# toposware/schnorr-sig

Hardware: AMD Instinct MI355X
Metric: Schnorr verifications/sec, 2^20-sig batch, 1/2/4/8 MI355X; bit-exact vs CPU (higher is better)
Workload: dtype u64

## Files before the change

### include/schnorr_sig_amd.h

```cpp
#ifndef SCHNORR_SIG_AMD_H
#define SCHNORR_SIG_AMD_H

#include <stddef.h>
#include <stdint.h>

#ifdef __cplusplus
extern "C" {
#endif

#define SSA_SIGNATURE_LENGTH 81
#define SSA_AFFINE_PK_LENGTH 96
#define SSA_SCALAR_LENGTH 32
#define SSA_PUBLIC_KEY_LENGTH 49
#define SSA_DIGEST_LENGTH 32
#define SSA_PARAMS_LENGTH 2816

#define SSA_OK 0
#define SSA_INVALID_PUBLIC_KEY 1
#define SSA_INVALID_SIGNATURE 2
#define SSA_MALFORMED 3

#define SSA_ERR_ARG (-1)
#define SSA_ERR_HIP (-2)
#define SSA_ERR_PARAMS (-3)
// ... 230 lines not shown

int ssa_multi_verify_batch_msm(ssa_multi *m, const uint8_t *sigs, const uint8_t *pks, const uint8_t *pk_inf,
                               const uint8_t *msgs, const uint64_t *msg_off, size_t msg_stride, size_t msg_len,
                               size_t n, const uint8_t *coeffs);

#define SSA_MSM_PARTIAL_WORDS 24
#define SSA_MSM_RECORD_MAGIC 0x5353415245430004ull
int ssa_verify_batch_msm_partial_device(ssa_ctx *ctx, const uint8_t *d_sigs, const uint8_t *d_pks,
                                        const uint8_t *d_pk_inf, const uint8_t *d_msgs, const uint64_t *d_msg_off,
                                        size_t msg_stride, size_t msg_len, size_t n, const uint8_t *d_coeffs,
                                        uint32_t coeff_bytes, uint64_t *d_partial_out);
int ssa_verify_batch_msm_partial(ssa_ctx *ctx, const uint8_t *sigs, const uint8_t *pks, const uint8_t *pk_inf,
                                 const uint8_t *msgs, const uint64_t *msg_off, size_t msg_stride, size_t msg_len,
                                 size_t n, const uint8_t *coeffs, uint64_t out24[SSA_MSM_PARTIAL_WORDS]);
int ssa_msm_combine_device(ssa_ctx *ctx, const uint64_t *d_parts24, size_t k, uint32_t *d_verdict_out);
int ssa_msm_combine(ssa_ctx *ctx, const uint64_t *parts24, size_t k);

#define SSA_ABI_VERSION 5
int ssa_abi_version(void);

int ssa_debug_arith(ssa_ctx *ctx, int op, const uint64_t *a, const uint64_t *b, size_t n,
                    size_t a_stride, size_t b_stride, uint64_t *out, size_t out_stride);
int ssa_debug_fault_after_chunk(ssa_ctx *ctx, int chunk);
int ssa_debug_table_read(ssa_ctx *ctx, int which, uint64_t first_row, uint64_t n, uint64_t *rows_out);
int ssa_debug_table_xor(ssa_ctx *ctx, int which, uint64_t row, uint32_t word, uint64_t mask);
int ssa_debug_corrupt_table_builds(int n);
int ssa_debug_keytab_xor(ssa_keyset *ks, ssa_keycache *kc, int what, uint64_t key, uint32_t word, uint64_t mask);
int ssa_debug_keytab_read(ssa_keyset *ks, ssa_keycache *kc, int what, uint64_t key, uint64_t *words_out);
int ssa_debug_tail_plan(unsigned waves, unsigned pieces, unsigned gens, int uniform, unsigned min_main, size_t n,
                        uint32_t flags, uint32_t out[14]);
int ssa_debug_screen_plan(size_t n, uint32_t coeff_bytes, uint64_t out[8]);
int ssa_debug_screen_segments(ssa_ctx *ctx, uint32_t k);
int ssa_debug_dedup_device(ssa_ctx *ctx, const uint8_t *d_pks, const uint8_t *d_pk_inf, size_t n,
                           uint32_t *d_key_idx_out, uint64_t out[2]);
int ssa_debug_dedup_config(ssa_ctx *ctx, double max_distinct_ratio, uint32_t probe_bound);
int ssa_debug_keycache_plan(uint64_t capacity, uint64_t held, uint64_t u, uint64_t m, uint32_t *plan_out);
int ssa_debug_chacha20(ssa_ctx *ctx, const uint8_t key[32], const uint8_t nonce[12], uint32_t counter0,
                       size_t n_blocks, uint8_t *out);
int ssa_bench_fpmul(ssa_ctx *ctx, int variant, double *fpmul_per_s);

#ifdef __cplusplus
}
#endif
#endif
```

### schnorr-sig_amd/__init__.py

```python
import ctypes as C
import os

import numpy as np

_HERE = os.path.dirname(os.path.abspath(__file__))
LIB_PATH = os.environ.get("SSA_LIB") or os.path.join(_HERE, "csrc", "libschnorr_sig_amd.so")

SCALAR_LENGTH = 32
PRIVATE_KEY_LENGTH = 32
BASEFIELD_LENGTH = 48
PUBLIC_KEY_LENGTH = 49
AFFINE_PUBLIC_KEY_LENGTH = 96
KEY_PAIR_LENGTH = 32
SIGNATURE_LENGTH = 81
KEYED_SIGNATURE_LENGTH = 130

OK, INVALID_PUBLIC_KEY, INVALID_SIGNATURE, MALFORMED = 0, 1, 2, 3
ERR_ARG, ERR_HIP, ERR_PARAMS, ERR_NO_DEVICE, ERR_TABLE = -1, -2, -3, -4, -5
TABLE_COMB, TABLE_CT = 0, 1
SELFCHECK_FIELDS = ("rows", "bad", "first_bad", "ctab_rows", "ctab_bad", "ctab_first_bad", "builds", "bits")
FLAG_CHECK_TORSION = 1
FLAG_FORCE_LANE = 2
FLAG_FORCE_COOP = 4
FLAG_SIG_FLAG_BYTE = 8
# ... 169 lines not shown
        "ssa_sign_many_indexed": (i32, [vp, vp, vp, vp, vp, vp, sz, sz, sz, u32, vp]),
        "ssa_sign_many_indexed_device": (i32, [vp, vp, vp, vp, vp, vp, sz, sz, sz, u32, vp, vp]),
        "ssa_ctx_selfcheck": (i32, [vp, u32, u64p]),
        "ssa_debug_table_read": (i32, [vp, i32, C.c_uint64, C.c_uint64, vp]),
        "ssa_debug_table_xor": (i32, [vp, i32, C.c_uint64, u32, C.c_uint64]),
        "ssa_debug_corrupt_table_builds": (i32, [i32]),
        "ssa_keyset_selfcheck": (i32, [vp, u32, vp, u64p]),
        "ssa_keycache_selfcheck": (i32, [vp, u32, u64p]),
        "ssa_debug_keytab_xor": (i32, [vp, vp, i32, C.c_uint64, u32, C.c_uint64]),
        "ssa_debug_keytab_read": (i32, [vp, vp, i32, C.c_uint64, vp]),
        "ssa_keygen_sign_many_rng": (i32, [vp, vp, vp, vp, sz, sz, sz, u32, vp, vp]),
        "ssa_keygen_sign_many_rng_device": (i32, [vp, vp, vp, vp, sz, sz, sz, u32, vp, vp]),
        "ssa_sign_many_indexed_rng": (i32, [vp, vp, vp, vp, vp, sz, sz, sz, u32, vp]),
        "ssa_sign_many_indexed_rng_device": (i32, [vp, vp, vp, vp, vp, sz, sz, sz, u32, vp, vp]),
        "ssa_signer_set_generate": (i32, [vp, sz, C.POINTER(vp)]),
        "ssa_signer_set_secret_keys": (i32, [vp, vp]),
        "ssa_debug_pin_rng": (i32, [vp, vp]),
        "ssa_debug_draw_scalars": (i32, [vp, vp, sz, vp]),
    }
    for name, (res, args) in sigs.items():
        fn = getattr(lib, name)
        fn.restype = res
        fn.argtypes = args
    got = lib.ssa_abi_version()
    if got != ABI_VERSION:
        raise ImportError("schnorr_sig_amd: %s has ABI version %d, this binding was written for %d -- rebuild "
                          "(python -c 'import __graft_entry__ as g; g.build(force=True)')" % (LIB_PATH, got, ABI_VERSION))
    return lib, list(sigs)


ABI_VERSION = 5
MSM_PARTIAL_WORDS = 24
MSM_RECORD_MAGIC = 0x5353415245430004
_lib, ABI_SYMBOLS = _load()


def _check(rc, what):
    if rc < 0:
        raise RuntimeError("%s failed: %s (%d)" % (what, _lib.ssa_strerror(rc).decode(), rc))
    return rc


def _np_u8(a, cols=None):
    a = np.ascontiguousarray(a, dtype=np.uint8)
    if cols is not None:
        a = a.reshape(-1, cols)
    return a


def _ptr(a):
    return None if a is None else C.c_void_p(a.ctypes.data)
# ... 573 lines not shown
        cnt = C.c_uint64(0)
        _check(_lib.ssa_ctx_read_timing(self._ctx, kernel.encode(), C.byref(avg), C.byref(cnt)),
               "ssa_ctx_read_timing")
        return avg.value, int(cnt.value)

    def host_path_probe(self, sigs_t, pks_t, msgs_t, n, reps=3):
        import time
        hs, hp, hm = (t[:n].cpu().numpy() for t in (sigs_t, pks_t, msgs_t))
        st, nf = self.verify_many(hs, hp, hm, check_torsion=False, mode="lane", sig_flag_byte=True)
        t0 = time.perf_counter()
        for _ in range(reps):
            st, nf = self.verify_many(hs, hp, hm, check_torsion=False, mode="lane", sig_flag_byte=True)
        dt = (time.perf_counter() - t0) / reps
        verdict = self.verify_batch_msm(hs, hp, hm)
        t0 = time.perf_counter()
        for _ in range(reps):
            verdict = self.verify_batch_msm(hs, hp, hm)
        dt_msm = (time.perf_counter() - t0) / reps
        return {"entry_point": "ssa_verify_many (host buffers in pageable memory, copied through the library's page-locked "
                               "bounce buffers, uploads in chunks overlapped with the hash kernel)",
                "ms_per_batch": dt * 1e3, "verifications_per_sec": n / dt, "rejected": int(nf),
                "verify_batch_msm_ms_per_batch": dt_msm * 1e3, "verify_batch_msm_signatures_per_sec": n / dt_msm,
                "verify_batch_msm_verdict": int(verdict)}

    def debug_arith(self, op, a, b, out_cols):
        a = np.ascontiguousarray(a, dtype=np.uint64)
        b = np.ascontiguousarray(b, dtype=np.uint64) if b is not None else None
        n = a.shape[0]
        out = np.zeros((n, out_cols), dtype=np.uint64)
        _check(_lib.ssa_debug_arith(self._ctx, op, _ptr(a), _ptr(b), n, a.shape[1],
                                    b.shape[1] if b is not None else 0, _ptr(out), out_cols), "ssa_debug_arith")
        return out

    def bench_fpmul(self, variant):
        v = C.c_double(0)
        _check(_lib.ssa_bench_fpmul(self._ctx, variant, C.byref(v)), "ssa_bench_fpmul")
        return v.value


def debug_corrupt_table_builds(n):
    _check(_lib.ssa_debug_corrupt_table_builds(int(n)), "ssa_debug_corrupt_table_builds")


KEYCHECK_DEEP, KEYCHECK_REPAIR = 1, 2
KEYCHECK_FIELDS = ("keys_checked", "keys_bad", "first_bad_key", "ladder_entries_checked", "comb_rows_checked",
                   "keys_rebuilt_and_compared", "combs_skipped", "rows_repaired")
# ... 193 lines not shown
        m = _np_u8(msgs)
        off = np.ascontiguousarray(offsets, dtype=np.uint64) if offsets is not None else None
        stride = mlen = 0 if off is not None else m.shape[1]
        inf = _np_u8(pk_inf) if pk_inf is not None else None
        c = _np_u8(coeffs, 32) if coeffs is not None else None
        return _check(_lib.ssa_multi_verify_batch_msm(self._m, _ptr(sigs), _ptr(pks), _ptr(inf), _ptr(m), _ptr(off),
                                                      stride, mlen, n, _ptr(c)), "ssa_multi_verify_batch_msm")


_default_engine = None


def debug_tail_plan(waves, n, check_torsion=False, pieces=5, gens=1, uniform=False, min_main=0):
    out = np.zeros(14, dtype=np.uint32)
    flags = 1 if check_torsion else 0
    _check(_lib.ssa_debug_tail_plan(int(waves), int(pieces), int(gens), int(bool(uniform)), int(min_main), int(n), flags,
                                    out.ctypes.data), "ssa_debug_tail_plan")

    def dec(d):
        d = int(d)
        return (d & 1, bool(d & 2), bool(d & 4), (d >> 8) & 0xff, (d >> 16) & 0xff)
    return {"n_pieces": int(out[0]), "tail_groups": int(out[1]), "main_blocks": int(out[2]), "grid_blocks": int(out[3]),
            "pieces": [dec(out[4 + k]) for k in range(int(out[0]))], "whole": [dec(out[12]), dec(out[13])]}


def debug_screen_plan(n, coeff_bytes=0):
    out = np.zeros(8, dtype=np.uint64)
    _check(_lib.ssa_debug_screen_plan(int(n), int(coeff_bytes), out.ctypes.data), "ssa_debug_screen_plan")
    keys = ("segments", "segment_lanes", "window_bits", "windows", "r_windows", "buckets_per_window", "slices",
            "total_segments")
    return {k: int(v) for k, v in zip(keys, out)}


def default_engine():
    global _default_engine
    if _default_engine is None:
        _default_engine = Engine(0)
    return _default_engine


class PublicKey:

    def __init__(self, affine96, is_identity=False):
        b = bytes(affine96)
        if len(b) != AFFINE_PUBLIC_KEY_LENGTH:
            raise ValueError("PublicKey needs 96 bytes of affine coordinates")
# ... 437 lines not shown
```

### schnorr-sig_amd/csrc/ssa_api.hip

```cpp
#define SSA_KERNELS_DEFINE 1
#include "ssa_ctx.hpp"
#include "ssa_keycache.hpp"

#include <sys/random.h>

#include <atomic>
#include <climits>
#include <functional>
#include <initializer_list>
#include <memory>
#include <mutex>
#include <thread>

static const unsigned char k_default_params[SSA_PARAMS_LENGTH] = {
#include "../params/params_default.inc"
};

extern "C" const char *ssa_strerror(int rc) {
    switch (rc) {
        case SSA_OK: return "ok";
        case SSA_INVALID_PUBLIC_KEY: return "The public key is not an element of the prime subgroup.";
        case SSA_INVALID_SIGNATURE: return "The signature is invalid or was incorrectly computed.";
        case SSA_MALFORMED: return "malformed input (the reference would panic)";
        case SSA_ERR_ARG: return "invalid argument";
// ... 136 lines not shown
    int v = 0;
    if (env_int(name, INT_MIN, INT_MAX, v) && std::find(set.begin(), set.end(), v) != set.end()) knob = (T)v;
}
static void env_flag(const char *name, bool &knob) {
    int v = 0;
    if (env_int(name, INT_MIN, INT_MAX, v)) knob = v != 0;
}

static void ctx_read_env(ssa_ctx *ctx, uint32_t *gtab_bits, uint64_t *hbm_budget_bytes) {
    CtxKnobs &k = ctx->knobs;
    if (env_u64("SSA_COOP_MAX_N", 0, UINT64_MAX, k.coop_max_n)) k.coop_max_n_torsion = k.coop_max_n;
    env_u64("SSA_MSM_SMALL_MAX", 0, UINT64_MAX, k.msm_small_max);
    env_one_of("SSA_VERIFY_BLOCK", {64, 128, 256}, k.verify_block);
    env_u64("SSA_LANE_SLICE", 256, UINT64_MAX, k.lane_slice);
    env_u64("SSA_MSM_SLICE", 256, (uint64_t)1 << 23, k.msm_slice);
    env_int("SSA_MSM_TREE_GROUP", 2, 64, k.msm_tree_group);
    env_int("SSA_TAIL_PIECES", 0, VP_MAX, k.tail_pieces);
    env_int("SSA_TAIL_GENS", 1, 8, k.tail_gens);
    env_flag("SSA_TAIL_UNIFORM", k.tail_uniform);
    env_int("SSA_TAIL_MIN_MAIN", INT_MIN, INT_MAX, k.tail_min_main);
    env_flag("SSA_TAIL_REVERSED", k.tail_reversed);
    env_int("SSA_TAIL_WAVES", INT_MIN, INT_MAX, k.tail_waves_override);
    env_flag("SSA_MSM_OVERLAP", k.msm_overlap);
    env_int("SSA_PIPELINE_CHUNKS", 1, 8, k.pipeline_chunks);
    env_flag("SSA_TWO_STREAMS", ctx->two_streams);
    uint64_t mb = 0;
    if (*hbm_budget_bytes == 0 && env_u64("SSA_HBM_BUDGET_MB", 0, UINT64_MAX, mb)) *hbm_budget_bytes = mb << 20;
    if (*gtab_bits == 0) env_one_of("SSA_GTAB_BITS", {16, 20, 22, 24}, *gtab_bits);
}

static int ctx_create(ssa_ctx **out, int device, const void *params, size_t params_len, uint32_t gtab_bits,
                      uint64_t hbm_budget_bytes, const CtxKnobs *inherit) {
    if (!out) return SSA_ERR_ARG;
    *out = nullptr;
    if (gtab_bits != 0 && gtab_bits != 16 && gtab_bits != 20 && gtab_bits != 22 && gtab_bits != 24) return SSA_ERR_ARG;
    int count = 0;
    if (hipGetDeviceCount(&count) != hipSuccess || count == 0) return SSA_ERR_NO_DEVICE;
    if (device < 0 || device >= count) return SSA_ERR_ARG;
    DevParams hp;
    if (params) {
        if (params_len != sizeof(DevParams)) return SSA_ERR_PARAMS;
        std::memcpy(&hp, params, sizeof hp);
    } else {
        std::memcpy(&hp, k_default_params, sizeof hp);
    }
    const bool is_default = std::memcmp(&hp, k_default_params, sizeof hp) == 0;
    if (int rc = validate_params(hp)) return rc;
    hp.flags = 0;
    bool small_mds = true;
    for (int i = 0; i < 144; i++) small_mds = small_mds && hp.mds[i] <= 0xffffffffull;
    if (small_mds) hp.flags |= PRM_FLAG_SMALL_MDS;
    bool tiny_mds = true;
    for (int i = 0; i < 144; i++) tiny_mds = tiny_mds && hp.mds[i] < 0x10000ull;
    if (tiny_mds) hp.flags |= PRM_FLAG_TINY_MDS;
    HIP_TRY(hipSetDevice(device));
    std::unique_ptr<ssa_ctx, decltype(&ssa_ctx_destroy)> guard(new ssa_ctx(), ssa_ctx_destroy);
    ssa_ctx *ctx = guard.get();
    ctx->device = device;
    ctx->default_params = is_default;
    if (inherit) ctx->knobs = *inherit;
    else ctx_read_env(ctx, &gtab_bits, &hbm_budget_bytes);
    HIP_TRY(hipStreamCreateWithFlags(&ctx->own_stream, hipStreamNonBlocking));
    HIP_TRY(hipStreamCreateWithFlags(&ctx->copy_stream, hipStreamNonBlocking));
    for (auto &st : ctx->hash_stream) HIP_TRY(hipStreamCreateWithFlags(&st, hipStreamNonBlocking));
    HIP_TRY(hipEventCreateWithFlags(&ctx->pipe_start, hipEventDisableTiming));
    HIP_TRY(hipEventCreateWithFlags(&ctx->order_ev, hipEventDisableTiming));
    for (int i = 0; i < 8; i++) {
        HIP_TRY(hipEventCreateWithFlags(&ctx->copy_done[i], hipEventDisableTiming));
        HIP_TRY(hipEventCreateWithFlags(&ctx->hash_done[i], hipEventDisableTiming));
    }
    ctx->stream = ctx->own_stream;
    if (!inherit) {
        hipDeviceProp_t prop;
        int occ = 0;
        if (hipGetDeviceProperties(&prop, device) == hipSuccess &&
            hipOccupancyMaxActiveBlocksPerMultiprocessor(&occ, ssa_k_verify, 256, 0) == hipSuccess && occ > 0)
            ctx->knobs.verify_waves = (unsigned)prop.multiProcessorCount * (unsigned)occ * 4u;
        (void)hipGetLastError();
        if (ctx->knobs.tail_waves_override) ctx->knobs.verify_waves = ctx->knobs.tail_waves_override;
    }
    HIP_TRY(hipMalloc((void **)&ctx->d_params, sizeof(DevParams)));
    HIP_TRY(hipMemcpy(ctx->d_params, &hp, sizeof hp, hipMemcpyHostToDevice));
    ctx->h_params = hp;
    if (hbm_budget_bytes == 0) {
        size_t free_b = 0, total_b = 0;
        if (hipMemGetInfo(&free_b, &total_b) != hipSuccess) free_b = 0;
        hbm_budget_bytes = free_b / 10;
    }
    ctx->hbm_budget = hbm_budget_bytes;
    static const u32 k_widths[4] = {24, 22, 20, 16};
    bool bad_table = false;
    for (u32 wbits : k_widths) {
        if (gtab_bits ? wbits > gtab_bits : (wbits > 16 && gtab_bytes(wbits) > hbm_budget_bytes)) continue;
// ... 14 lines not shown
    *out = guard.release();
    return 0;
}

extern "C" int ssa_ctx_create_ex(ssa_ctx **out, int device, const void *params, size_t params_len, uint32_t gtab_bits,
                                 uint64_t hbm_budget_bytes) {
    return ctx_create(out, device, params, params_len, gtab_bits, hbm_budget_bytes, nullptr);
}

extern "C" int ssa_ctx_create(ssa_ctx **out, int device, const void *params, size_t params_len) {
    return ssa_ctx_create_ex(out, device, params, params_len, 0u, 0ull);
}

ssa_ctx *ssa_internal_twin(ssa_ctx *ctx) {
    if (ctx->is_twin || !ctx->two_streams) return nullptr;
    if (!ctx->twin) {
        DevParams hp = ctx->h_params;
        hp.flags = 0;
        if (ctx_create(&ctx->twin, ctx->device, &hp, sizeof hp, ctx->gtab_bits, ctx->hbm_budget, &ctx->knobs) != 0) {
            ctx->two_streams = false;
            return nullptr;
        }
        ctx->twin->is_twin = true;
    }
    ctx->twin->knobs = ctx->knobs;
    return ctx->twin;
}

template <class T, class F>
static void orphan_handles(std::vector<T *> &v, F &&release) {
    for (T *h : v) {
        release(h);
        h->ctx = nullptr;
    }
    v.clear();
}

extern "C" void ssa_ctx_destroy(ssa_ctx *ctx) {
    if (!ctx) return;
    (void)hipSetDevice(ctx->device);
    if (ctx->stream) (void)hipStreamSynchronize(ctx->stream);
    if (ctx->twin) {
        ssa_ctx_destroy(ctx->twin);
        ctx->twin = nullptr;
    }
    orphan_handles(ctx->keysets, [](ssa_keyset *ks) { ks->release_all(); });
    orphan_handles(ctx->signer_sets, [](ssa_signer_set *ss) { ss->wipe_release(); });
    orphan_handles(ctx->keycaches, [](ssa_keycache *kc) { kc->release_all(); });
    for (auto &kv : ctx->timed)
        for (auto &t : kv.second) {
            (void)hipEventDestroy(t.start);
            (void)hipEventDestroy(t.stop);
        }
    for_each_devbuf(ctx, [](DevBuf &b) { b.release(); });
    for_each_hostbuf(ctx, [](HostBuf &b) { b.release(); });
    if (ctx->d_params) (void)hipFree(ctx->d_params);
    gtab_release(ctx->gtab_share);
    ctx->gtab_share = nullptr;
    ctx->d_gtab = nullptr;
    for (auto &ev : ctx->copy_done)
        if (ev) (void)hipEventDestroy(ev);
    for (auto &ev : ctx->hash_done)
        if (ev) (void)hipEventDestroy(ev);
    if (ctx->pipe_start) (void)hipEventDestroy(ctx->pipe_start);
    if (ctx->order_ev) (void)hipEventDestroy(ctx->order_ev);
    for (auto &st : ctx->hash_stream)
        if (st) (void)hipStreamDestroy(st);
    if (ctx->copy_stream) (void)hipStreamDestroy(ctx->copy_stream);
// ... 1063 lines not shown
            std::vector<uint64_t> off;
            const HostBatch s = b.slice(lo, cnt, off);
            rcs[r] = ssa_verify_batch_msm_partial(m->ctxs[r], s.sigs, s.pks, s.pk_inf, s.msgs, s.msg_off, msg_stride, msg_len,
                                                  cnt, coeffs ? coeffs + 32 * lo : nullptr, &parts[24 * r]);
        });
    }
    for (auto &t : threads) t.join();
    for (size_t r = 0; r < world; r++)
        if (rcs[r] != 0) return rcs[r];
    return ssa_msm_combine(m->ctxs[0], parts.data(), world);
}

extern "C" int ssa_debug_corrupt_table_builds(int n) {
    if (n < 0) return SSA_ERR_ARG;
    g_corrupt_builds.store(n);
    return 0;
}

extern "C" int ssa_debug_fault_after_chunk(ssa_ctx *ctx, int chunk) {
    if (!ctx) return SSA_ERR_ARG;
    ctx->fault_after_chunk = chunk;
    return 0;
}

extern "C" int ssa_debug_arith(ssa_ctx *ctx, int op, const uint64_t *a, const uint64_t *b, size_t n,
                               size_t a_stride, size_t b_stride, uint64_t *out, size_t out_stride) {
    if (!ctx || !a || !out || n == 0 || op < 0 || op > 18) return SSA_ERR_ARG;
    if ((op == 0 || op == 3 || op == 4 || op == 5 || (op >= 7 && op != 18)) && !b) return SSA_ERR_ARG;
    if (op == 18 && (a_stride < 2 || out_stride < 6)) return SSA_ERR_ARG;
    if (op >= 15 && op <= 17) {
        if (a_stride < 20 || b_stride < 12 || out_stride < 19) return SSA_ERR_ARG;
        if (op != 16)
            for (size_t i = 0; i < n; i++)
                if (a[i * a_stride + 19] == 0 || a[i * a_stride + 19] > 64 || a[i * a_stride + 19] != a[19])
                    return SSA_ERR_ARG;
    }
    HostCall hc(ctx);
    const u64 *da = hc.in<u64>(ctx->st_aux, a, n * a_stride * 8), *db = b ? hc.in<u64>(ctx->st_aux2, b, n * b_stride * 8) : nullptr;
    u64 *d_out = (u64 *)hc.out(ctx->st_status, out, n * out_stride * 8);
    return hc.finish([&] {
        HIP_TRY(hipMemsetAsync(d_out, 0, n * out_stride * 8, ctx->stream));
        if (op == 7) {
            hipLaunchKernelGGL(ssa_k_debug_coop, dim3((unsigned)n), dim3(64), 0, ctx->stream, da, db, n, a_stride, b_stride,
                               d_out, out_stride);
        } else if (op == 4 || (op >= 15 && op <= 17)) {
            if (ctx->ws_tab.reserve(n * (size_t)(PTAB_ENTRIES * PTAB_ENTRY_U64) * sizeof(u64))) return SSA_ERR_HIP;
// ... 100 lines not shown
```

### schnorr-sig_amd/csrc/ssa_ctx.hpp

```cpp
#pragma once
#include "../../include/schnorr_sig_amd.h"
#include "ssa_kernels.hpp"

#include <hip/hip_runtime.h>

#include <algorithm>
#include <cstdio>
#include <cstdlib>
#include <cstring>
#include <map>
#include <mutex>
#include <string>
#include <thread>
#include <utility>
#include <vector>

using namespace ssa;

static inline bool ssa_debug_enabled() {
    static const bool on = std::getenv("SSA_DEBUG") != nullptr;
    return on;
}
#define HIP_TRY(expr)                                                                    \
    do {                                                                                 \
// ... 49 lines not shown
            (void)hipGetLastError();
            p = nullptr;
            return SSA_ERR_HIP;
        }
        cap = want;
        return 0;
    }
    void release() {
        if (p) (void)hipHostFree(p);
        p = nullptr;
        cap = 0;
    }
};

struct TimedLaunch {
    hipEvent_t start, stop;
};

constexpr double DEDUP_RATIO_NO_CHECK = 0.0, DEDUP_RATIO_CHECK = 1.0;
constexpr unsigned DEDUP_PROBE_BOUND = 128;

struct CtxKnobs {
    size_t pipeline_min_n = 1 << 17;
    unsigned pipeline_chunks = 8;
    size_t coop_max_n = 7680, coop_max_n_torsion = 10496;
    size_t msm_small_max = 3072;
    size_t lane_slice = (size_t)1 << 20, msm_slice = (size_t)1 << 23;
    bool msm_overlap = true;
    unsigned msm_tree_group = 16;
    unsigned verify_block = 256;
    unsigned verify_waves = 0;
    unsigned tail_pieces = 5;
    unsigned tail_gens = 1;
    bool tail_uniform = false;
    bool tail_reversed = false;
    unsigned tail_min_main = 0;
    unsigned tail_waves_override = 0;
    bool timing = false;
    unsigned screen_segs = 0;
    double dedup_ratio[2] = {DEDUP_RATIO_NO_CHECK, DEDUP_RATIO_CHECK};
    unsigned dedup_probe_bound = DEDUP_PROBE_BOUND;
};

#define SSA_CTX_DEVBUFS(X) \
    X(ws_h) X(ws_tab) X(ws_fail) \
     \
    X(st_sigs) X(st_pks) X(st_inf) X(st_msgs) X(st_off) X(st_status) X(st_aux) X(st_aux2) X(st_coeffs) \
// ... 8 lines not shown
     \
    X(scr_mask) X(scr_mark) X(scr_list) X(scr_blk) X(scr_cnt) \
     \
    X(dd_slots) X(dd_rep) X(dd_num) X(dd_reps) X(dd_idx) X(dd_blk) X(dd_stats) X(dd_pks) X(dd_inf) X(dd_kstatus) \
     \
    X(kc_found) X(kc_missrep) X(kc_blk) X(kc_lane_row) \
     \
    X(ctab) X(sg_sigs) X(sg_pks) \
    X(tc_out)            \
    X(kck_ws)            \
    X(dv_recs)           \
     \
    X(rng_seed) X(rng_scratch) \
     \
    X(tail_done) X(tail_park)

#define SSA_CTX_HOSTBUFS(X) X(pin_in) X(pin_coeffs) X(pin_out) X(pin_seed)

struct ssa_ctx {
    int device = 0;
    hipStream_t own_stream = nullptr;
    hipStream_t stream = nullptr;
    hipStream_t copy_stream = nullptr;
    hipEvent_t copy_done[8] = {};
    hipStream_t hash_stream[2] = {};
    hipEvent_t hash_done[8] = {};
    hipEvent_t pipe_start = nullptr;
    hipEvent_t order_ev = nullptr;
    CtxKnobs knobs;
    DevParams *d_params = nullptr;
    u64 *d_gtab = nullptr;
    struct SharedGtab *gtab_share = nullptr;
    uint32_t gtab_bits = 0;
    uint64_t hbm_budget = 0;
    DevParams h_params;
    ssa_ctx *twin = nullptr;
    bool is_twin = false, two_streams = true;
#define X(name) DevBuf name;
    SSA_CTX_DEVBUFS(X)
#undef X
#define X(name) HostBuf name;
    SSA_CTX_HOSTBUFS(X)
#undef X
    bool default_params = false;
    int fault_after_chunk = -1;
    uint64_t dedup_key[2] = {0, 0};
    bool dedup_key_set = false;
    bool ctab_ready = false;
    bool rng_pinned = false;
    uint8_t rng_pin[44] = {};
    std::map<std::string, std::vector<TimedLaunch>> timed;
    std::vector<struct ssa_keyset *> keysets;
    std::vector<struct ssa_signer_set *> signer_sets;
    std::vector<struct ssa_keycache *> keycaches;
};

template <class Ctx, class F>
static inline void for_each_devbuf(Ctx *c, F &&f) {
#define X(name) f(c->name);
    SSA_CTX_DEVBUFS(X)
// ... 272 lines not shown
        settled = rc == 0;
        return rc;
    }
};


int ssa_internal_hash_chunk(ssa_ctx *ctx, hipStream_t hs, const DevBatch &b, size_t cnt, uint64_t *d_h);

struct SideStreamDrain {
    ssa_ctx *armed = nullptr;
    void done() { armed = nullptr; }
    ~SideStreamDrain() {
        if (!armed) return;
        (void)hipStreamSynchronize(armed->copy_stream);
        for (auto &hs : armed->hash_stream) (void)hipStreamSynchronize(hs);
        (void)hipStreamSynchronize(armed->stream);
    }
};

struct PipelinedInputs : SideStreamDrain {
    StagedInputs s;
};

static inline size_t host_copy_threads() {
    static const size_t t = [] {
        const char *e = std::getenv("SSA_COPY_THREADS");
        const long v = e ? std::atol(e) : 8;
        return (size_t)(v < 1 ? 1 : v > 32 ? 32 : v);
    }();
    return t;
}
static inline void host_copy(void *dst, const void *src, size_t bytes) {
    constexpr size_t PIECE = 4u << 20;
    if (bytes <= 2 * PIECE || host_copy_threads() == 1) {
        std::memcpy(dst, src, bytes);
        return;
    }
    const size_t parts = bytes / PIECE < host_copy_threads() ? bytes / PIECE : host_copy_threads();
    const size_t per = (bytes / parts + 63) & ~(size_t)63;
    std::vector<std::thread> th;
    for (size_t t = 1; t < parts; t++) {
        const size_t lo = t * per, hi = t + 1 == parts ? bytes : (t + 1) * per;
        th.emplace_back([=] { std::memcpy((char *)dst + lo, (const char *)src + lo, hi - lo); });
    }
    std::memcpy(dst, src, per < bytes ? per : bytes);
    for (auto &x : th) x.join();
}

static inline int pipeline_fault_chunk(ssa_ctx *ctx) {
    const int k = ctx->fault_after_chunk;
    ctx->fault_after_chunk = -1;
    return k;
}

static inline int pipelined_upload_hash(ssa_ctx *ctx, const HostBatch &b, size_t n, PipelinedInputs &pin, bool *used) {
    const uint8_t *sigs = b.sigs, *pks = b.pks, *pk_inf = b.pk_inf, *msgs = b.msgs;
    const uint64_t *msg_off = b.msg_off;
    const size_t msg_stride = b.msg_stride, msg_len = b.msg_len;
    *used = false;
    const size_t mb = msgs_bytes(msg_off, msg_stride, msg_len, n);
    if (mb && !msgs) return SSA_ERR_ARG;
    auto al = [](size_t b) { return (b + 255) & ~(size_t)255; };
    const size_t o_pks = al(n * 81), o_msgs = o_pks + al(n * 96), o_inf = o_msgs + al(mb),
                 o_off = o_inf + al(pk_inf ? n : 0), total = o_off + al(msg_off ? (n + 1) * sizeof(uint64_t) : 0);
    if (ctx->pin_in.reserve(total)) return 0;
    u8 *h_sigs = (u8 *)ctx->pin_in.p, *h_pks = h_sigs + o_pks, *h_msgs = h_sigs + o_msgs, *h_inf = h_sigs + o_inf,
       *h_off = h_sigs + o_off;
    *used = true;
    if (ctx->st_sigs.reserve(n * 81) || ctx->st_pks.reserve(n * 96) || ctx->st_msgs.reserve(mb + 16) ||
        ctx->ws_h.reserve(n * 4 * sizeof(u64)) || (msg_off && ctx->st_off.reserve((n + 1) * sizeof(uint64_t))) ||
        (pk_inf && ctx->st_inf.reserve(n)))
        return SSA_ERR_HIP;
    HIP_TRY(hipEventRecord(ctx->pipe_start, ctx->stream));
    HIP_TRY(hipStreamWaitEvent(ctx->copy_stream, ctx->pipe_start, 0));
    for (auto &hs : ctx->hash_stream) HIP_TRY(hipStreamWaitEvent(hs, ctx->pipe_start, 0));
    pin.armed = ctx;
    const int fault_chunk = pipeline_fault_chunk(ctx);
    u8 *d_sigs = (u8 *)ctx->st_sigs.p, *d_pks = (u8 *)ctx->st_pks.p, *d_msgs = (u8 *)ctx->st_msgs.p;
    DevBatch &d = pin.s.batch;
    d = {d_sigs, d_pks, nullptr, {d_msgs, nullptr, msg_stride, msg_len}};
    if (msg_off) {
        host_copy(h_off, msg_off, (n + 1) * sizeof(uint64_t));
        HIP_TRY(hipMemcpyAsync(ctx->st_off.p, h_off, (n + 1) * sizeof(uint64_t), hipMemcpyHostToDevice, ctx->copy_stream));
        d.msgs.off = (const u64 *)ctx->st_off.p;
    }
    if (pk_inf) {
        host_copy(h_inf, pk_inf, n);
        HIP_TRY(hipMemcpyAsync(ctx->st_inf.p, h_inf, n, hipMemcpyHostToDevice, ctx->copy_stream));
        d.pk_inf = (const u8 *)ctx->st_inf.p;
    }
    const unsigned chunks = ctx->knobs.pipeline_chunks;
    for (unsigned c = 0; c < chunks; c++) {
        const size_t lo = n * c / chunks, hi = n * (c + 1) / chunks, cnt = hi - lo;
        if (cnt == 0) continue;
        host_copy(h_sigs + 81 * lo, sigs + 81 * lo, cnt * 81);
        HIP_TRY(hipMemcpyAsync(d_sigs + 81 * lo, h_sigs + 81 * lo, cnt * 81, hipMemcpyHostToDevice, ctx->copy_stream));
        host_copy(h_pks + 96 * lo, pks + 96 * lo, cnt * 96);
        HIP_TRY(hipMemcpyAsync(d_pks + 96 * lo, h_pks + 96 * lo, cnt * 96, hipMemcpyHostToDevice, ctx->copy_stream));
        const size_t m_lo = msg_off ? (size_t)msg_off[lo] : lo * msg_stride;
        const size_t m_hi = msg_off ? (size_t)msg_off[hi] : (hi == n ? mb : hi * msg_stride);
        if (m_hi > m_lo) {
            host_copy(h_msgs + m_lo, msgs + m_lo, m_hi - m_lo);
            HIP_TRY(hipMemcpyAsync(d_msgs + m_lo, h_msgs + m_lo, m_hi - m_lo, hipMemcpyHostToDevice, ctx->copy_stream));
        }
        HIP_TRY(hipEventRecord(ctx->copy_done[c], ctx->copy_stream));
        hipStream_t hs = ctx->hash_stream[c & 1u];
        HIP_TRY(hipStreamWaitEvent(hs, ctx->copy_done[c], 0));
        if (int rc = ssa_internal_hash_chunk(ctx, hs, d.slice(lo), cnt, (uint64_t *)ctx->ws_h.p + 4 * lo)) return rc;
        HIP_TRY(hipEventRecord(ctx->hash_done[c], hs));
        HIP_TRY(hipStreamWaitEvent(ctx->stream, ctx->hash_done[c], 0));
        if ((int)c == fault_chunk) return SSA_ERR_HIP;
    }
    return 0;
}

static inline StagedInputs slice_inputs(HostCall &hc, PipelinedInputs &pin, const HostBatch &b, size_t n,
                                        const uint8_t *coeffs, bool pipeline, bool pin_out) {
    ssa_ctx *ctx = hc.ctx;
    if (hc.ok() && pipeline && n >= ctx->knobs.pipeline_min_n && ctx->knobs.pipeline_chunks > 1 && !(pin_out && ctx->pin_out.reserve(n)) &&
        (!coeffs || ctx->pin_coeffs.reserve(n * 32) == 0)) {
        bool used = false;
        if (coeffs && ctx->st_coeffs.reserve(n * 32)) hc.rc = SSA_ERR_HIP;
        else hc.rc = pipelined_upload_hash(ctx, b, n, pin, &used);
        if (!hc.ok() || used) {
            StagedInputs s = pin.s;
            s.hashed = true;
            if (coeffs && hc.ok()) {
                host_copy(ctx->pin_coeffs.p, coeffs, n * 32);
                hc.step([&] {
                    HIP_TRY(hipMemcpyAsync(ctx->st_coeffs.p, ctx->pin_coeffs.p, n * 32, hipMemcpyHostToDevice, ctx->copy_stream));
                    HIP_TRY(hipEventRecord(ctx->pipe_start, ctx->copy_stream));
                    HIP_TRY(hipStreamWaitEvent(ctx->stream, ctx->pipe_start, 0));
                    return 0;
                });
                s.coeffs = (const u8 *)ctx->st_coeffs.p;
            }
            return s;
        }
    }
    StagedInputs s;
    s.batch.sigs = hc.in(ctx->st_sigs, b.sigs, n * 81);
    s.batch.pks = hc.in(ctx->st_pks, b.pks, n * 96);
    if (b.pk_inf) s.batch.pk_inf = hc.in(ctx->st_inf, b.pk_inf, n);
    s.batch.msgs = hc.msgs(b.msgs, b.msg_off, b.msg_stride, b.msg_len, n);
    if (coeffs) s.coeffs = hc.in(ctx->st_coeffs, coeffs, n * 32);
    return s;
}

template <class F>
static int status_host_one(ssa_ctx *ctx, const HostBatch &b, size_t n, const uint8_t *coeffs, bool pipeline, bool pin_out,
                           uint8_t *status_out, uint64_t *n_fail_out, F &&device_form) {
    HostCall hc(ctx);
    PipelinedInputs pin;
    const StagedInputs s = slice_inputs(hc, pin, b, n, coeffs, pipeline, pin_out);
    const bool through_pin = pin_out && s.hashed;
    u8 *d_status = hc.out(ctx->st_status, through_pin ? ctx->pin_out.p : status_out, n, 16);
    unsigned long long nf = 0, *d_fail = (unsigned long long *)ctx->ws_fail.p;
    hc.copy_back(&nf, d_fail, sizeof nf);
    if (int rc = hc.finish([&] { return device_form(s, d_status, d_fail); })) return rc;
// ... 89 lines not shown
```

Measured before the change: 30.61 million.

## Overlap host staging copies with uploads via persistent copy pool and ramped chunk plan

Replaces the per-call spawn-and-join threaded host memcpy with a persistent worker pool. All chunks' pageable-to-pinned copies are posted up front, so later chunks are staged while earlier chunks upload and hash. The uniform 8-chunk split becomes a plan with small, doubling leading chunks followed by 8 body chunks, which gets the first hash kernel started sooner. Coefficient and offset uploads are also chunked into the same pipeline. The cost is persistent threads, lock contention on a shared queue, and more HIP calls per batch.

```diff
diff --git a/include/schnorr_sig_amd.h b/include/schnorr_sig_amd.h
--- a/include/schnorr_sig_amd.h
+++ b/include/schnorr_sig_amd.h
@@ -276,6 +276,12 @@
 int ssa_debug_arith(ssa_ctx *ctx, int op, const uint64_t *a, const uint64_t *b, size_t n,
                     size_t a_stride, size_t b_stride, uint64_t *out, size_t out_stride);
 int ssa_debug_fault_after_chunk(ssa_ctx *ctx, int chunk);
+int ssa_debug_upload_plan(size_t n, uint32_t explicit_chunks, size_t first_lanes, uint64_t out[20]);
+int ssa_debug_copy_pool_create(void **pool_out);
+int ssa_debug_copy_pool_copy(void *pool, uint32_t threads, void *dst, const void *src, size_t bytes);
+int ssa_debug_copy_pool_workers(void *pool);
+void ssa_debug_copy_pool_destroy(void *pool);
+int ssa_debug_copy_workers(ssa_ctx *ctx);
 int ssa_debug_table_read(ssa_ctx *ctx, int which, uint64_t first_row, uint64_t n, uint64_t *rows_out);
 int ssa_debug_table_xor(ssa_ctx *ctx, int which, uint64_t row, uint32_t word, uint64_t mask);
 int ssa_debug_corrupt_table_builds(int n);
diff --git a/schnorr-sig_amd/__init__.py b/schnorr-sig_amd/__init__.py
--- a/schnorr-sig_amd/__init__.py
+++ b/schnorr-sig_amd/__init__.py
@@ -215,11 +215,26 @@
         fn = getattr(lib, name)
         fn.restype = res
         fn.argtypes = args
+    later = {
+        "ssa_debug_upload_plan": (i32, [sz, u32, sz, vp]),
+        "ssa_debug_copy_pool_create": (i32, [C.POINTER(vp)]),
+        "ssa_debug_copy_pool_copy": (i32, [vp, u32, vp, vp, sz]),
+        "ssa_debug_copy_pool_workers": (i32, [vp]),
+        "ssa_debug_copy_pool_destroy": (None, [vp]),
+        "ssa_debug_copy_workers": (i32, [vp]),
+    }
+    bound = list(sigs)
+    for name, (res, args) in later.items():
+        fn = getattr(lib, name, None)
+        if fn is not None:
+            fn.restype = res
+            fn.argtypes = args
+            bound.append(name)
     got = lib.ssa_abi_version()
     if got != ABI_VERSION:
         raise ImportError("schnorr_sig_amd: %s has ABI version %d, this binding was written for %d -- rebuild "
                           "(python -c 'import __graft_entry__ as g; g.build(force=True)')" % (LIB_PATH, got, ABI_VERSION))
-    return lib, list(sigs)
+    return lib, bound
 
 
 ABI_VERSION = 5
@@ -839,6 +854,9 @@
                 "ms_per_batch": dt * 1e3, "verifications_per_sec": n / dt, "rejected": int(nf),
                 "verify_batch_msm_ms_per_batch": dt_msm * 1e3, "verify_batch_msm_signatures_per_sec": n / dt_msm,
                 "verify_batch_msm_verdict": int(verdict)}
+
+    def debug_copy_workers(self):
+        return _check(_lib.ssa_debug_copy_workers(self._ctx), "ssa_debug_copy_workers")
 
     def debug_arith(self, op, a, b, out_cols):
         a = np.ascontiguousarray(a, dtype=np.uint64)
@@ -1078,6 +1096,37 @@
         return (d & 1, bool(d & 2), bool(d & 4), (d >> 8) & 0xff, (d >> 16) & 0xff)
     return {"n_pieces": int(out[0]), "tail_groups": int(out[1]), "main_blocks": int(out[2]), "grid_blocks": int(out[3]),
             "pieces": [dec(out[4 + k]) for k in range(int(out[0]))], "whole": [dec(out[12]), dec(out[13])]}
+
+
+def debug_upload_plan(n, chunks=0, first_lanes=0):
+    out = np.zeros(20, dtype=np.uint64)
+    _check(_lib.ssa_debug_upload_plan(int(n), int(chunks), int(first_lanes), out.ctypes.data), "ssa_debug_upload_plan")
+    k = int(out[0])
+    return {"bounds": [int(v) for v in out[3:4 + k]] if k else [], "ramp": int(out[1]), "pipeline_min_n": int(out[2])}
+
+
+class DebugCopyPool:
+
+    def __init__(self, threads=8):
+        self._pool = C.c_void_p()
+        self.threads = int(threads)
+        _check(_lib.ssa_debug_copy_pool_create(C.byref(self._pool)), "ssa_debug_copy_pool_create")
+
+    def copy(self, dst, src, nbytes=None):
+        nbytes = src.nbytes if nbytes is None else int(nbytes)
+        assert nbytes <= src.nbytes and nbytes <= dst.nbytes
+        _check(_lib.ssa_debug_copy_pool_copy(self._pool, self.threads, dst.ctypes.data, src.ctypes.data, nbytes),
+               "ssa_debug_copy_pool_copy")
+
+    def workers(self):
+        return _check(_lib.ssa_debug_copy_pool_workers(self._pool), "ssa_debug_copy_pool_workers")
+
+    def close(self):
+        if self._pool:
+            _lib.ssa_debug_copy_pool_destroy(self._pool)
+            self._pool = C.c_void_p()
+
+    __del__ = close
 
 
 def debug_screen_plan(n, coeff_bytes=0):
diff --git a/schnorr-sig_amd/csrc/ssa_api.hip b/schnorr-sig_amd/csrc/ssa_api.hip
--- a/schnorr-sig_amd/csrc/ssa_api.hip
+++ b/schnorr-sig_amd/csrc/ssa_api.hip
@@ -182,7 +182,9 @@
     env_flag("SSA_TAIL_REVERSED", k.tail_reversed);
     env_int("SSA_TAIL_WAVES", INT_MIN, INT_MAX, k.tail_waves_override);
     env_flag("SSA_MSM_OVERLAP", k.msm_overlap);
-    env_int("SSA_PIPELINE_CHUNKS", 1, 8, k.pipeline_chunks);
+    env_int("SSA_PIPELINE_CHUNKS", 1, (int)UPLOAD_MAX_CHUNKS, k.pipeline_chunks);
+    env_u64("SSA_PIPELINE_FIRST", 256, (uint64_t)1 << 20, k.pipeline_first);
+    env_int("SSA_COPY_THREADS", 1, 32, k.copy_threads);
     env_flag("SSA_TWO_STREAMS", ctx->two_streams);
     uint64_t mb = 0;
     if (*hbm_budget_bytes == 0 && env_u64("SSA_HBM_BUDGET_MB", 0, UINT64_MAX, mb)) *hbm_budget_bytes = mb << 20;
@@ -225,10 +227,8 @@
     for (auto &st : ctx->hash_stream) HIP_TRY(hipStreamCreateWithFlags(&st, hipStreamNonBlocking));
     HIP_TRY(hipEventCreateWithFlags(&ctx->pipe_start, hipEventDisableTiming));
     HIP_TRY(hipEventCreateWithFlags(&ctx->order_ev, hipEventDisableTiming));
-    for (int i = 0; i < 8; i++) {
-        HIP_TRY(hipEventCreateWithFlags(&ctx->copy_done[i], hipEventDisableTiming));
-        HIP_TRY(hipEventCreateWithFlags(&ctx->hash_done[i], hipEventDisableTiming));
-    }
+    for (auto &ev : ctx->copy_done) HIP_TRY(hipEventCreateWithFlags(&ev, hipEventDisableTiming));
+    for (auto &ev : ctx->hash_done) HIP_TRY(hipEventCreateWithFlags(&ev, hipEventDisableTiming));
     ctx->stream = ctx->own_stream;
     if (!inherit) {
         hipDeviceProp_t prop;
@@ -289,6 +289,7 @@
             return nullptr;
         }
         ctx->twin->is_twin = true;
+        ctx->twin->pool = &ctx->own_pool;
     }
     ctx->twin->knobs = ctx->knobs;
     return ctx->twin;
@@ -311,6 +312,7 @@
         ssa_ctx_destroy(ctx->twin);
         ctx->twin = nullptr;
     }
+    ctx->own_pool.shutdown();
     orphan_handles(ctx->keysets, [](ssa_keyset *ks) { ks->release_all(); });
     orphan_handles(ctx->signer_sets, [](ssa_signer_set *ss) { ss->wipe_release(); });
     orphan_handles(ctx->keycaches, [](ssa_keycache *kc) { kc->release_all(); });
@@ -1420,6 +1422,32 @@
     ctx->fault_after_chunk = chunk;
     return 0;
 }
+
+extern "C" int ssa_debug_upload_plan(size_t n, uint32_t explicit_chunks, size_t first_lanes, uint64_t out[20]) {
+    if (!out || explicit_chunks > UPLOAD_MAX_CHUNKS) return SSA_ERR_ARG;
+    const UploadPlan p = upload_plan(n, explicit_chunks, first_lanes);
+    out[0] = p.chunks;
+    out[1] = p.ramp;
+    out[2] = CtxKnobs().pipeline_min_n;
+    for (unsigned c = 0; c <= UPLOAD_MAX_CHUNKS; c++) out[3 + c] = c <= p.chunks ? p.bound[c] : 0;
+    return 0;
+}
+
+extern "C" int ssa_debug_copy_pool_create(void **pool_out) {
+    if (!pool_out) return SSA_ERR_ARG;
+    *pool_out = new CopyPool();
+    return 0;
+}
+extern "C" int ssa_debug_copy_pool_copy(void *pool, uint32_t threads, void *dst, const void *src, size_t bytes) {
+    if (!pool || threads < 1 || threads > 32 || (bytes && (!dst || !src))) return SSA_ERR_ARG;
+    CopyJob job;
+    ((CopyPool *)pool)->post(job, dst, src, bytes, threads);
+    job.wait();
+    return 0;
+}
+extern "C" int ssa_debug_copy_pool_workers(void *pool) { return pool ? (int)((CopyPool *)pool)->workers() : SSA_ERR_ARG; }
+extern "C" void ssa_debug_copy_pool_destroy(void *pool) { delete (CopyPool *)pool; }
+extern "C" int ssa_debug_copy_workers(ssa_ctx *ctx) { return ctx ? (int)ctx->pool->workers() : SSA_ERR_ARG; }
 
 extern "C" int ssa_debug_arith(ssa_ctx *ctx, int op, const uint64_t *a, const uint64_t *b, size_t n,
                                size_t a_stride, size_t b_stride, uint64_t *out, size_t out_stride) {
diff --git a/schnorr-sig_amd/csrc/ssa_copy_pool.hpp b/schnorr-sig_amd/csrc/ssa_copy_pool.hpp
--- /dev/null
+++ b/schnorr-sig_amd/csrc/ssa_copy_pool.hpp
@@ -0,0 +1,158 @@
+#pragma once
+
+#include <condition_variable>
+#include <cstddef>
+#include <cstring>
+#include <deque>
+#include <mutex>
+#include <thread>
+#include <vector>
+
+struct CopyPool;
+
+struct CopyJob {
+    CopyPool *pool = nullptr;
+    size_t pending = 0;
+    CopyJob() = default;
+    CopyJob(const CopyJob &) = delete;
+    CopyJob &operator=(const CopyJob &) = delete;
+    inline void wait();
+    inline ~CopyJob();
+};
+
+struct CopyPool {
+    static constexpr size_t PIECE = (size_t)1 << 20;
+    static constexpr size_t INLINE_MAX = (size_t)64 << 10;
+    struct Piece {
+        char *dst;
+        const char *src;
+        size_t bytes;
+        CopyJob *job;
+    };
+    std::mutex mu;
+    std::condition_variable work, done;
+    std::deque<Piece> q;
+    std::vector<std::thread> th;
+    bool stop = false;
+
+    CopyPool() = default;
+    CopyPool(const CopyPool &) = delete;
+    CopyPool &operator=(const CopyPool &) = delete;
+    ~CopyPool() { shutdown(); }
+
+    void post(CopyJob &job, void *dst, const void *src, size_t bytes, unsigned threads) {
+        if (bytes == 0) return;
+        if (bytes > INLINE_MAX) {
+            std::unique_lock<std::mutex> lk(mu);
+            if (th.empty()) start_locked(threads);
+            if (!th.empty()) {
+                job.pool = this;
+                for (size_t lo = 0; lo < bytes; lo += PIECE) {
+                    q.push_back({(char *)dst + lo, (const char *)src + lo, bytes - lo < PIECE ? bytes - lo : PIECE, &job});
+                    job.pending++;
+                }
+                lk.unlock();
+                work.notify_all();
+                return;
+            }
+        }
+        std::memcpy(dst, src, bytes);
+    }
+    void wait(CopyJob &job) {
+        std::unique_lock<std::mutex> lk(mu);
+        done.wait(lk, [&] { return job.pending == 0; });
+    }
+    void cancel(CopyJob &job) {
+        std::unique_lock<std::mutex> lk(mu);
+        if (job.pending == 0) return;
+        for (auto it = q.begin(); it != q.end();) {
+            if (it->job == &job) {
+                it = q.erase(it);
+                job.pending--;
+            } else {
+                ++it;
+            }
+        }
+        done.wait(lk, [&] { return job.pending == 0; });
+    }
+    void shutdown() {
+        {
+            std::lock_guard<std::mutex> lk(mu);
+            if (th.empty()) return;
+            stop = true;
+        }
+        work.notify_all();
+        for (auto &t : th) t.join();
+        std::lock_guard<std::mutex> lk(mu);
+        th.clear();
+        stop = false;
+    }
+    size_t workers() {
+        std::lock_guard<std::mutex> lk(mu);
+        return th.size();
+    }
+
+  private:
+    void start_locked(unsigned threads) {
+        threads = threads < 1 ? 1 : threads > 32 ? 32 : threads;
+        try {
+            for (unsigned t = 0; t < threads; t++) th.emplace_back([this] { run(); });
+        } catch (...) {
+        }
+    }
+    void run() {
+        std::unique_lock<std::mutex> lk(mu);
+        for (;;) {
+            work.wait(lk, [&] { return stop || !q.empty(); });
+            if (q.empty()) return;
+            const Piece p = q.front();
+            q.pop_front();
+            lk.unlock();
+            std::memcpy(p.dst, p.src, p.bytes);
+            lk.lock();
+            if (--p.job->pending == 0) done.notify_all();
+        }
+    }
+};
+
+inline void CopyJob::wait() {
+    if (pool) pool->wait(*this);
+}
+inline CopyJob::~CopyJob() {
+    if (pool) pool->cancel(*this);
+}
+
+constexpr unsigned UPLOAD_MAX_CHUNKS = 16;
+constexpr unsigned UPLOAD_BODY_CHUNKS = 8;
+constexpr size_t UPLOAD_FIRST_LANES = 8192;
+struct UploadPlan {
+    unsigned chunks = 0, ramp = 0;
+    size_t bound[UPLOAD_MAX_CHUNKS + 1] = {};
+};
+
+static inline UploadPlan upload_plan(size_t n, unsigned explicit_chunks, size_t first_lanes) {
+    UploadPlan p;
+    auto cut = [&](size_t b) {
+        if (b > p.bound[p.chunks] && p.chunks < UPLOAD_MAX_CHUNKS) p.bound[++p.chunks] = b;
+    };
+    if (n == 0) return p;
+    if (explicit_chunks) {
+        const size_t k = explicit_chunks > UPLOAD_MAX_CHUNKS ? UPLOAD_MAX_CHUNKS : explicit_chunks;
+        for (size_t c = 1; c < k; c++) cut((n * c / k) & ~(size_t)255);
+        cut(n);
+        return p;
+    }
+    const size_t u = n / 256;
+    size_t s = (first_lanes ? first_lanes : UPLOAD_FIRST_LANES) / 256, sum = 0;
+    if (s == 0) s = 1;
+    while (p.chunks < UPLOAD_MAX_CHUNKS - UPLOAD_BODY_CHUNKS && s * (UPLOAD_BODY_CHUNKS + 1) <= u - sum) {
+        sum += s;
+        cut(256 * sum);
+        s *= 2;
+    }
+    p.ramp = p.chunks;
+    const size_t rest = u - sum;
+    for (size_t c = 1; c < UPLOAD_BODY_CHUNKS; c++) cut(256 * (sum + rest * c / UPLOAD_BODY_CHUNKS));
+    cut(n);
+    return p;
+}
diff --git a/schnorr-sig_amd/csrc/ssa_ctx.hpp b/schnorr-sig_amd/csrc/ssa_ctx.hpp
--- a/schnorr-sig_amd/csrc/ssa_ctx.hpp
+++ b/schnorr-sig_amd/csrc/ssa_ctx.hpp
@@ -1,5 +1,6 @@
 #pragma once
 #include "../../include/schnorr_sig_amd.h"
+#include "ssa_copy_pool.hpp"
 #include "ssa_kernels.hpp"
 
 #include <hip/hip_runtime.h>
@@ -95,7 +96,9 @@
 
 struct CtxKnobs {
     size_t pipeline_min_n = 1 << 17;
-    unsigned pipeline_chunks = 8;
+    unsigned pipeline_chunks = 0;
+    size_t pipeline_first = UPLOAD_FIRST_LANES;
+    unsigned copy_threads = 8;
     size_t coop_max_n = 7680, coop_max_n_torsion = 10496;
     size_t msm_small_max = 3072;
     size_t lane_slice = (size_t)1 << 20, msm_slice = (size_t)1 << 23;
@@ -150,9 +153,9 @@
     hipStream_t own_stream = nullptr;
     hipStream_t stream = nullptr;
     hipStream_t copy_stream = nullptr;
-    hipEvent_t copy_done[8] = {};
+    hipEvent_t copy_done[UPLOAD_MAX_CHUNKS] = {};
     hipStream_t hash_stream[2] = {};
-    hipEvent_t hash_done[8] = {};
+    hipEvent_t hash_done[UPLOAD_MAX_CHUNKS] = {};
     hipEvent_t pipe_start = nullptr;
     hipEvent_t order_ev = nullptr;
     CtxKnobs knobs;
@@ -164,6 +167,8 @@
     DevParams h_params;
     ssa_ctx *twin = nullptr;
     bool is_twin = false, two_streams = true;
+    CopyPool own_pool;
+    CopyPool *pool = &own_pool;
 #define X(name) DevBuf name;
     SSA_CTX_DEVBUFS(X)
 #undef X
@@ -482,38 +487,14 @@
     StagedInputs s;
 };
 
-static inline size_t host_copy_threads() {
-    static const size_t t = [] {
-        const char *e = std::getenv("SSA_COPY_THREADS");
-        const long v = e ? std::atol(e) : 8;
-        return (size_t)(v < 1 ? 1 : v > 32 ? 32 : v);
-    }();
-    return t;
-}
-static inline void host_copy(void *dst, const void *src, size_t bytes) {
-    constexpr size_t PIECE = 4u << 20;
-    if (bytes <= 2 * PIECE || host_copy_threads() == 1) {
-        std::memcpy(dst, src, bytes);
-        return;
-    }
-    const size_t parts = bytes / PIECE < host_copy_threads() ? bytes / PIECE : host_copy_threads();
-    const size_t per = (bytes / parts + 63) & ~(size_t)63;
-    std::vector<std::thread> th;
-    for (size_t t = 1; t < parts; t++) {
-        const size_t lo = t * per, hi = t + 1 == parts ? bytes : (t + 1) * per;
-        th.emplace_back([=] { std::memcpy((char *)dst + lo, (const char *)src + lo, hi - lo); });
-    }
-    std::memcpy(dst, src, per < bytes ? per : bytes);
-    for (auto &x : th) x.join();
-}
-
 static inline int pipeline_fault_chunk(ssa_ctx *ctx) {
     const int k = ctx->fault_after_chunk;
     ctx->fault_after_chunk = -1;
     return k;
 }
 
-static inline int pipelined_upload_hash(ssa_ctx *ctx, const HostBatch &b, size_t n, PipelinedInputs &pin, bool *used) {
+static inline int pipelined_upload_hash(ssa_ctx *ctx, const HostBatch &b, size_t n, const uint8_t *coeffs,
+                                        PipelinedInputs &pin, bool *used) {
     const uint8_t *sigs = b.sigs, *pks = b.pks, *pk_inf = b.pk_inf, *msgs = b.msgs;
     const uint64_t *msg_off = b.msg_off;
     const size_t msg_stride = b.msg_stride, msg_len = b.msg_len;
@@ -524,8 +505,9 @@
     const size_t o_pks = al(n * 81), o_msgs = o_pks + al(n * 96), o_inf = o_msgs + al(mb),
                  o_off = o_inf + al(pk_inf ? n : 0), total = o_off + al(msg_off ? (n + 1) * sizeof(uint64_t) : 0);
     if (ctx->pin_in.reserve(total)) return 0;
-    u8 *h_sigs = (u8 *)ctx->pin_in.p, *h_pks = h_sigs + o_pks, *h_msgs = h_sigs + o_msgs, *h_inf = h_sigs + o_inf,
-       *h_off = h_sigs + o_off;
+    u8 *h_sigs = (u8 *)ctx->pin_in.p, *h_pks = h_sigs + o_pks, *h_msgs = h_sigs + o_msgs, *h_inf = h_sigs + o_inf;
+    u64 *h_off = (u64 *)(h_sigs + o_off);
+    u8 *h_coeffs = (u8 *)ctx->pin_coeffs.p;
     *used = true;
     if (ctx->st_sigs.reserve(n * 81) || ctx->st_pks.reserve(n * 96) || ctx->st_msgs.reserve(mb + 16) ||
         ctx->ws_h.reserve(n * 4 * sizeof(u64)) || (msg_off && ctx->st_off.reserve((n + 1) * sizeof(uint64_t))) ||
@@ -537,39 +519,60 @@
     pin.armed = ctx;
     const int fault_chunk = pipeline_fault_chunk(ctx);
     u8 *d_sigs = (u8 *)ctx->st_sigs.p, *d_pks = (u8 *)ctx->st_pks.p, *d_msgs = (u8 *)ctx->st_msgs.p;
+    u8 *d_inf = (u8 *)ctx->st_inf.p, *d_coeffs = (u8 *)ctx->st_coeffs.p;
+    u64 *d_off = (u64 *)ctx->st_off.p;
     DevBatch &d = pin.s.batch;
-    d = {d_sigs, d_pks, nullptr, {d_msgs, nullptr, msg_stride, msg_len}};
-    if (msg_off) {
-        host_copy(h_off, msg_off, (n + 1) * sizeof(uint64_t));
-        HIP_TRY(hipMemcpyAsync(ctx->st_off.p, h_off, (n + 1) * sizeof(uint64_t), hipMemcpyHostToDevice, ctx->copy_stream));
-        d.msgs.off = (const u64 *)ctx->st_off.p;
-    }
-    if (pk_inf) {
-        host_copy(h_inf, pk_inf, n);
-        HIP_TRY(hipMemcpyAsync(ctx->st_inf.p, h_inf, n, hipMemcpyHostToDevice, ctx->copy_stream));
-        d.pk_inf = (const u8 *)ctx->st_inf.p;
-    }
-    const unsigned chunks = ctx->knobs.pipeline_chunks;
-    for (unsigned c = 0; c < chunks; c++) {
-        const size_t lo = n * c / chunks, hi = n * (c + 1) / chunks, cnt = hi - lo;
-        if (cnt == 0) continue;
-        host_copy(h_sigs + 81 * lo, sigs + 81 * lo, cnt * 81);
-        HIP_TRY(hipMemcpyAsync(d_sigs + 81 * lo, h_sigs + 81 * lo, cnt * 81, hipMemcpyHostToDevice, ctx->copy_stream));
-        host_copy(h_pks + 96 * lo, pks + 96 * lo, cnt * 96);
-        HIP_TRY(hipMemcpyAsync(d_pks + 96 * lo, h_pks + 96 * lo, cnt * 96, hipMemcpyHostToDevice, ctx->copy_stream));
+    d = {d_sigs, d_pks, pk_inf ? d_inf : nullptr, {d_msgs, msg_off ? d_off : nullptr, msg_stride, msg_len}};
+
+    const UploadPlan plan = upload_plan(n, ctx->knobs.pipeline_chunks, ctx->knobs.pipeline_first);
+    struct Span {
+        size_t lo, cnt, o_lo, o_cnt, m_lo, m_cnt;
+    };
+    auto span = [&](unsigned c) {
+        const size_t lo = plan.bound[c], hi = plan.bound[c + 1];
+        const size_t o_lo = c == 0 ? 0 : lo + 1;
         const size_t m_lo = msg_off ? (size_t)msg_off[lo] : lo * msg_stride;
         const size_t m_hi = msg_off ? (size_t)msg_off[hi] : (hi == n ? mb : hi * msg_stride);
-        if (m_hi > m_lo) {
-            host_copy(h_msgs + m_lo, msgs + m_lo, m_hi - m_lo);
-            HIP_TRY(hipMemcpyAsync(d_msgs + m_lo, h_msgs + m_lo, m_hi - m_lo, hipMemcpyHostToDevice, ctx->copy_stream));
-        }
+        return Span{lo, hi - lo, o_lo, hi + 1 - o_lo, m_lo, m_hi - m_lo};
+    };
+    struct ChunkJobs {
+        CopyJob off, inf, sigs, pks, msgs, coeffs;
+    } jobs[UPLOAD_MAX_CHUNKS];
+    CopyPool &pool = *ctx->pool;
+    const unsigned workers = ctx->knobs.copy_threads;
+    for (unsigned c = 0; c < plan.chunks; c++) {
+        const Span sp = span(c);
+        if (msg_off) pool.post(jobs[c].off, h_off + sp.o_lo, msg_off + sp.o_lo, sp.o_cnt * sizeof(uint64_t), workers);
+        if (pk_inf) pool.post(jobs[c].inf, h_inf + sp.lo, pk_inf + sp.lo, sp.cnt, workers);
+        pool.post(jobs[c].sigs, h_sigs + 81 * sp.lo, sigs + 81 * sp.lo, sp.cnt * 81, workers);
+        pool.post(jobs[c].pks, h_pks + 96 * sp.lo, pks + 96 * sp.lo, sp.cnt * 96, workers);
+        pool.post(jobs[c].msgs, h_msgs + sp.m_lo, msgs + sp.m_lo, sp.m_cnt, workers);
+        if (coeffs) pool.post(jobs[c].coeffs, h_coeffs + 32 * sp.lo, coeffs + 32 * sp.lo, sp.cnt * 32, workers);
+    }
+    auto upload = [&](CopyJob &job, void *dst, const void *src, size_t bytes) {
+        job.wait();
+        if (bytes == 0) return hipSuccess;
+        return hipMemcpyAsync(dst, src, bytes, hipMemcpyHostToDevice, ctx->copy_stream);
+    };
+    for (unsigned c = 0; c < plan.chunks; c++) {
+        const Span sp = span(c);
+        if (msg_off) HIP_TRY(upload(jobs[c].off, d_off + sp.o_lo, h_off + sp.o_lo, sp.o_cnt * sizeof(uint64_t)));
+        if (pk_inf) HIP_TRY(upload(jobs[c].inf, d_inf + sp.lo, h_inf + sp.lo, sp.cnt));
+        HIP_TRY(upload(jobs[c].sigs, d_sigs + 81 * sp.lo, h_sigs + 81 * sp.lo, sp.cnt * 81));
+        HIP_TRY(upload(jobs[c].pks, d_pks + 96 * sp.lo, h_pks + 96 * sp.lo, sp.cnt * 96));
+        HIP_TRY(upload(jobs[c].msgs, d_msgs + sp.m_lo, h_msgs + sp.m_lo, sp.m_cnt));
         HIP_TRY(hipEventRecord(ctx->copy_done[c], ctx->copy_stream));
         hipStream_t hs = ctx->hash_stream[c & 1u];
         HIP_TRY(hipStreamWaitEvent(hs, ctx->copy_done[c], 0));
-        if (int rc = ssa_internal_hash_chunk(ctx, hs, d.slice(lo), cnt, (uint64_t *)ctx->ws_h.p + 4 * lo)) return rc;
+        if (int rc = ssa_internal_hash_chunk(ctx, hs, d.slice(sp.lo), sp.cnt, (uint64_t *)ctx->ws_h.p + 4 * sp.lo)) return rc;
         HIP_TRY(hipEventRecord(ctx->hash_done[c], hs));
         HIP_TRY(hipStreamWaitEvent(ctx->stream, ctx->hash_done[c], 0));
+        if (coeffs) HIP_TRY(upload(jobs[c].coeffs, d_coeffs + 32 * sp.lo, h_coeffs + 32 * sp.lo, sp.cnt * 32));
         if ((int)c == fault_chunk) return SSA_ERR_HIP;
+    }
+    if (coeffs) {
+        HIP_TRY(hipEventRecord(ctx->pipe_start, ctx->copy_stream));
+        HIP_TRY(hipStreamWaitEvent(ctx->stream, ctx->pipe_start, 0));
     }
     return 0;
 }
@@ -577,24 +580,15 @@
 static inline StagedInputs slice_inputs(HostCall &hc, PipelinedInputs &pin, const HostBatch &b, size_t n,
                                         const uint8_t *coeffs, bool pipeline, bool pin_out) {
     ssa_ctx *ctx = hc.ctx;
-    if (hc.ok() && pipeline && n >= ctx->knobs.pipeline_min_n && ctx->knobs.pipeline_chunks > 1 && !(pin_out && ctx->pin_out.reserve(n)) &&
+    if (hc.ok() && pipeline && n >= ctx->knobs.pipeline_min_n && ctx->knobs.pipeline_chunks != 1 && !(pin_out && ctx->pin_out.reserve(n)) &&
         (!coeffs || ctx->pin_coeffs.reserve(n * 32) == 0)) {
         bool used = false;
         if (coeffs && ctx->st_coeffs.reserve(n * 32)) hc.rc = SSA_ERR_HIP;
-        else hc.rc = pipelined_upload_hash(ctx, b, n, pin, &used);
+        else hc.rc = pipelined_upload_hash(ctx, b, n, coeffs, pin, &used);
         if (!hc.ok() || used) {
             StagedInputs s = pin.s;
             s.hashed = true;
-            if (coeffs && hc.ok()) {
-                host_copy(ctx->pin_coeffs.p, coeffs, n * 32);
-                hc.step([&] {
-                    HIP_TRY(hipMemcpyAsync(ctx->st_coeffs.p, ctx->pin_coeffs.p, n * 32, hipMemcpyHostToDevice, ctx->copy_stream));
-                    HIP_TRY(hipEventRecord(ctx->pipe_start, ctx->copy_stream));
-                    HIP_TRY(hipStreamWaitEvent(ctx->stream, ctx->pipe_start, 0));
-                    return 0;
-                });
-                s.coeffs = (const u8 *)ctx->st_coeffs.p;
-            }
+            if (coeffs && hc.ok()) s.coeffs = (const u8 *)ctx->st_coeffs.p;
             return s;
         }
     }
```

New measurement: 30.60 million (median of 2 runs). No clear change (-0.0%).
